# Arshardh/siddhi

Hardware: AMD Instinct MI355X
Metric: events/sec (node) windowed group-by agg at 1/2/4/8 GPUs; % HBM roofline (higher is better)
Workload: dtype f64; 1 GPU; C2 timeBatch(1 sec) count/min/max/avg group by k, per-event sends; key_type=string (dictionary ids = dense slots), keys_per_gpu=100000, keys_total=100000, send_size=1, parallelism=key-sharded x1, flushes=69793, rows=6978983088

## Files before the change

### siddhi_amd/csrc/sh_kernels.hip

```cpp
#include "sh_device.h"

namespace shd {

#ifdef SH_STAMPS
constexpr int kStampKernels = 4, kStampBlocks = 32768, kStampPts = 16;
__device__ unsigned long long g_stamps[kStampKernels * kStampBlocks * kStampPts];
#define SH_STAMP(kern, pt)                                                                                   \
    do {                                                                                                     \
        if (threadIdx.x == 0 && blockIdx.x < kStampBlocks) {                                                 \
            asm volatile("s_waitcnt vmcnt(0) lgkmcnt(0)" ::: "memory");                                      \
            g_stamps[((size_t)(kern) * kStampBlocks + blockIdx.x) * kStampPts + (pt)] = __builtin_amdgcn_s_memtime(); \
        }                                                                                                    \
    } while (0)
#else
#define SH_STAMP(kern, pt) do {} while (0)
#endif

template <int FK>
__global__ __launch_bounds__(kBlock) void k_blockagg(const i64* __restrict__ ts, ColSet cols, FilterProg f,
                                                    WinParams wp, i64* blk_pass, i64* blk_tl, i64* blk_first,
                                                    i64* blk_xm) {
    i64 base = (i64)blockIdx.x * kTile + (i64)threadIdx.x * kItems;
    i64 cnt = 0, tl = INT64_MIN, first = INT64_MAX, xm = INT64_MIN;
    i64 tsv[kItems];
// ... 224 lines not shown
                ms_counts[(i64)(ms_col0 + tile) * P + i] = mhist[i];
        }
    }
    i64 cnt = 0, tl = INT64_MIN;
    SendCursor sc(wp, base);
#pragma unroll
    for (int i = 0; i < kItems; i++) {
        i64 e = base + i;
        bool in = e < wp.N;
        cnt += pass[i];
        if (!SORTED && in && sc.last(wp, e)) tl = max(tl, t[i]);
        sc.next();
    }
    i64 pcb, pm = INT64_MIN;
    if (SORTED) {
        i64 tot_c;
        pcb = block_excl_scan(cnt, SumOp(), 0, &tot_c);
        if (threadIdx.x == 0) blk_pass_pre[tile] = tot_c;
        bool down = false;
#pragma unroll
        for (int i = 0; i + 1 < kItems; i++) down |= base + i + 1 < wp.N && t[i + 1] < t[i];
        if (base + kItems < wp.N) down |= ts[base + kItems] < t[kItems - 1];
        if (down) atomicOr(&info->unsorted, 1);
    } else {
        pcb = block_excl_scan(cnt, SumOp(), 0, nullptr) + blk_pass_pre[tile];
        pm = max(block_excl_scan(tl, MaxOp(), INT64_MIN, nullptr), blk_tl_pre[tile]);
    }
    constexpr bool ext = EXT;
    i64 av[kItems];
    i64 M = INT64_MIN;
    if (ext) {
        load_items_raw(cols, wp.ts_col, base, wp.N, av);
        i64 xm = INT64_MIN;
// ... 86 lines not shown
    int* nb = &info->n_bounds;
#define SH_BOUNDS(EXT, FK, S)                                                                                     \
    hipLaunchKernelGGL((k_boundaries<EXT, FK, S>), dim3(nblk), dim3(kBlock), lds, s, ts, cols, f, wp, blk_pass_pre, \
                       blk_tl_pre, info, bounds, max_bounds, nb, kp, kt, new_pos, blk_xm_pre, ms_counts, P, ms_nblk,   \
                       ms_col0)
    const int fk = filter_kind(f);
    if (wp.kind == SH_WIN_EXT_TIME_BATCH) SH_BOUNDS(true, 2, false);
    else if (sorted) {
        if (fk == 0) SH_BOUNDS(false, 0, true);
        else if (fk == 1) SH_BOUNDS(false, 1, true);
        else SH_BOUNDS(false, 2, true);
    } else if (fk == 0) SH_BOUNDS(false, 0, false);
    else if (fk == 1) SH_BOUNDS(false, 1, false);
    else SH_BOUNDS(false, 2, false);
#undef SH_BOUNDS
    if (sorted) {
        launch_scan_sum_large(s, blk_pass_pre, nblk + 1, scan_tmp);
        hipLaunchKernelGGL(k_fix_bounds, dim3(1), dim3(kBlock), 0, s, bounds, max_bounds, blk_pass_pre, nblk, ts, wp,
                           info);
    }
}

struct AggLds {
    u64* fields;
    u32* cnt;
    u32* first;
    u32* last;
    u32* owner;
};


// ... 1748 lines not shown
```

### siddhi_amd/csrc/sh_runtime.cpp

```cpp
#include <hip/hip_runtime.h>

#include <algorithm>
#include <cstdio>
#include <cstdlib>
#include <cstring>
#include <string>
#include <vector>

#include "sh_agg.h"
#include "sh_internal.h"
#include "sh_runtime.h"

#include <chrono>

using namespace shd;

thread_local std::string g_last_error;

int sh_fail(int code, const std::string& msg) {
    g_last_error = msg;
    SH_TRACE("error %d: %s", code, msg.c_str());
    return code;
}

// ... 128 lines not shown
    HIPCHK(hipSetDevice(device));
    hipDeviceProp_t prop;
    HIPCHK(hipGetDeviceProperties(&prop, device));
    if (std::string(prop.gcnArchName).find("gfx950") == std::string::npos)
        return sh_fail(SH_ERR_DEVICE, std::string("built for gfx950, found ") + prop.gcnArchName);
    hipMemPool_t pool = nullptr;
    if (hipDeviceGetDefaultMemPool(&pool, device) == hipSuccess && pool) {
        uint64_t keep = UINT64_MAX;
        (void)hipMemPoolSetAttribute(pool, hipMemPoolAttrReleaseThreshold, &keep);
    }
    sh_ctx* c = new sh_ctx();
    c->device = device;
    c->num_cus = prop.multiProcessorCount;
    c->max_lds = (int)prop.sharedMemPerBlock;
    if (hipStreamCreateWithFlags(&c->stream, hipStreamNonBlocking) != hipSuccess ||
        hipStreamCreateWithFlags(&c->copy_stream, hipStreamNonBlocking) != hipSuccess) {
        if (c->stream) (void)hipStreamDestroy(c->stream);
        delete c;
        return sh_fail(SH_ERR_DEVICE, "hipStreamCreate failed");
    }
    *out = c;
    return SH_OK;
}

extern "C" int sh_ctx_destroy(sh_ctx* c) {
    if (!c) return SH_OK;
    (void)hipStreamSynchronize(c->stream);
    (void)hipStreamSynchronize(c->copy_stream);
    (void)hipStreamDestroy(c->stream);
    (void)hipStreamDestroy(c->copy_stream);
    delete c;
    return SH_OK;
}

extern "C" int sh_alloc_pinned(int64_t bytes, void** out) {
    if (!out || bytes < 0) return sh_fail(SH_ERR_INVALID, "sh_alloc_pinned: bad arguments");
    HIPCHK(hipHostMalloc(out, (size_t)std::max<int64_t>(bytes, 1), hipHostMallocDefault));
    return SH_OK;
}

extern "C" int sh_free_pinned(void* p) {
    if (p) HIPCHK(hipHostFree(p));
    return SH_OK;
}

extern "C" const char* sh_last_error(void) { return g_last_error.c_str(); }
extern "C" int32_t sh_abi_version(void) { return SH_ABI_VERSION; }

Tuning Tuning::from_env() {
    Tuning t;
    auto on = [](const char* n) { const char* v = getenv(n); return v && *v && strcmp(v, "0") != 0; };
    t.direct_pos = on("SH_DIRECT_POS");
    t.part_keys_1024 = getenv("SH_PART_KEYS") && atoi(getenv("SH_PART_KEYS")) == 1024;
    t.no_async_small = on("SH_NO_ASYNC_SMALL");
    t.sl_records_seq = !getenv("SH_SL_RECORDS_SEQ") || on("SH_SL_RECORDS_SEQ");
    t.pl_sort = !getenv("SH_PL_SORT") || on("SH_PL_SORT");
    if (getenv("SH_AGG_BAND_ROWS")) t.agg_band_rows = atoi(getenv("SH_AGG_BAND_ROWS"));
    t.slx_wave = !getenv("SH_SLX_WAVE") || on("SH_SLX_WAVE");
    return t;
}

extern "C" int sh_query_set_strings(sh_query* q, int32_t col, int64_t first_id, int64_t n, const uint16_t* units,
                                    const int64_t* offsets) {
    if (!q) return sh_fail(SH_ERR_INVALID, "sh_query_set_strings: NULL query");
    if (col < 0 || col >= q->d.n_cols || q->d.col_types[col] != SH_T_STRID)
        return sh_fail(SH_ERR_INVALID, "sh_query_set_strings: not a string column");
    if (first_id < 0 || n < 0 || first_id + n > ((int64_t)1 << 31) || (n > 0 && (!units || !offsets)))
        return sh_fail(SH_ERR_INVALID, "sh_query_set_strings: bad id range");
    for (int64_t i = 0; i < n; i++)
        if (offsets[i + 1] < offsets[i] || offsets[i] < 0)
            return sh_fail(SH_ERR_INVALID, "sh_query_set_strings: offsets must be non-decreasing");
    auto& v = q->strings[col];
    auto& set = q->strings_set[col];
// ... 212 lines not shown
```

### siddhi_amd/csrc/sh_runtime.h

```cpp
#pragma once

#include <hip/hip_runtime.h>
#include <rocprofiler-sdk-roctx/roctx.h>

#include <algorithm>
#include <cstdio>
#include <new>
#include <utility>
#include <string>
#include <unordered_map>
#include <vector>

#include "sh_internal.h"
#include "sh_having.h"

struct sh_ctx {
    int device = 0;
    int num_cus = 0;
    int max_lds = 0;
    hipStream_t stream = nullptr;
    hipStream_t copy_stream = nullptr;
};

int sh_fail(int code, const std::string& msg);

bool sh_trace_on();
#define SH_TRACE(...)                                    \
    do {                                                 \
        if (sh_trace_on()) {                             \
            fprintf(stderr, "[sh] " __VA_ARGS__);        \
            fputc('\n', stderr);                         \
            fflush(stderr);                              \
        }                                                \
    } while (0)

bool sh_timing_on();
// ... 150 lines not shown
    DevBuf blk;
    int stage(hipStream_t s, const sh_batch* b, int n_cols, const int32_t* types, sh_batch* dev);
};

size_t type_size(int t);

using shd::AggPlan;
using shd::FilterProg;
using shd::KeyPlan;
using shd::PushInfo;
using shd::TileMap;

struct SlidingImpl;

struct Tuning {
    bool direct_pos = false, part_keys_1024 = false, no_async_small = false, sl_records_seq = false;
    bool pl_sort = true;
    bool slx_wave = true;
    int agg_band_rows = 8;
    static Tuning from_env();
};

struct WideKeys;
struct sh_query {
    int kind = 0;
    Tuning tune = Tuning::from_env();
    SlidingImpl* sl = nullptr;
    std::unordered_map<int, std::vector<std::u16string>> strings;
    std::unordered_map<int, std::vector<char>> strings_set;
    bool partitioned = false, p0_known = false;
// ... 37 lines not shown
    DevBuf fl_dev;
    HavingState hv;
    std::vector<std::pair<int64_t, int64_t>> xr_starts;
    std::vector<int64_t> xr_rep, xr_vals;
    bool xt_Lvalid = false;
    int64_t xt_L = 0;
    int64_t xt_nnew = 0;
    DevBuf sc_slp, sc_fflag, sc_fo, sc_fc, sc_bclk;
    DevBuf xt_dev;
    PinnedBuf xt_host;
    int64_t n_pend = 0, pend_cap = 0;
    int64_t last_nb = 0;
    int64_t seq = 0;
    DevBuf pend_pos, pend_ts, pend_vals;
    DevBuf pend_tmp;
    DevBuf blk_pass, blk_tl, blk_first, blk_xm, info, bounds, segs, seg_rows, rows, counters, out_ts, out_keys, out_vals,
        out_nulls, out_expired, out_rep, blk_cnt;
    DevBuf first_bits, word_pre;
    DevBuf emit_stage;
    const void* zeroed_nulls = nullptr;
    const void* zeroed_expired = nullptr;
    DevBuf ms_counts, ms_tmp, rec_pos, rec_idx, rec_vals, part_off;
    DevBuf new_pos, seg_off;
    PushInfo* h_info = nullptr;
    PinnedBuf h_up;
    PinnedBuf h_tail;
    PinnedBuf h_bounds;
    bool ms_ready = false;
    bool rec_packed = false;
    bool direct_pos = false;
// ... 18 lines not shown
    int64_t rec_cap = 0;
    struct ClosedTail {
        bool active = false, host_done = false;
        int nseg = 0, units_per_seg = 1;
        int64_t closed_hi = 0;
        std::vector<int64_t> clocks, windows;
    } tail;
    StagedBatch staged;
    OutHost out;
    sh_out dev_out{};
    PinnedVec<int64_t> dev_flush_offsets{0}, dev_flush_clock;
    hipEvent_t ev_push0 = nullptr, ev_push1 = nullptr, ev_agg0 = nullptr, ev_agg1 = nullptr;
    hipEvent_t ev_srt0 = nullptr, ev_srt1 = nullptr;
    bool srt_timed = false;
    hipEvent_t ev_mid = nullptr;
    sh_stats stats{};
    int64_t agg_bytes = 0;
    std::vector<int64_t> flush_window;
    bool internal_keys = false;
    size_t kt_min_size = 0;
    int32_t load_type[SH_MAX_COLS]{};
    uint32_t cols_used = 0;
    bool given = false;
    const int* given_wcol = nullptr;
    const shd::u64* given_gidx = nullptr;
    const int64_t* given_clk = nullptr;
    int64_t given_seq0 = 0, given_ss = 1;
    int64_t given_W_base = 0, given_W_end = 0;
    std::vector<sh_bound> gbounds;
    DevBuf pend_gidx, out_order;
// ... 73 lines not shown
struct FlushVecs {
    PinnedVec<int64_t>& offsets;
    PinnedVec<int64_t>& clocks;
};
inline FlushVecs flush_vecs(sh_query* q, bool host_out) {
    if (host_out) return {q->out.flush_offsets, q->out.flush_clock};
    return {q->dev_flush_offsets, q->dev_flush_clock};
}

int sc_rows(sh_query* q, const sh_batch* b, const std::vector<shd::Bound>& bounds, int64_t n_old, int64_t M, bool cv0,
            int64_t clock0, int64_t seq0, bool host_out);
int sc_expire_pending(sh_query* q, int64_t now, bool host_out);
int hv_closed(sh_query* q, const std::vector<shd::Segment>& segs, const std::vector<int64_t>& clocks, const sh_batch* b,
              bool host_out);
int append_pending(sh_query* q, const sh_batch* b, int64_t n_old, int64_t M);
int upload_segments(sh_query* q, const std::vector<shd::Segment>& segs);

int partition_filter(const FilterProg& base, int pcol, int ptype, int64_t key, FilterProg* out);

int64_t given_flush_clock(const sh_query* q, int64_t W);
int query_push_given(sh_query* q, const sh_batch* b, bool host_out, const sh_out** out);
int query_close_given(sh_query* q, bool host_out, const sh_out** out);
int query_advance(sh_query* q, int64_t now, bool host_out, const sh_out** out);

int query_reserve_keys(sh_query* q, int64_t extra);
int query_drain_async(sh_query* q);
int query_swap_keys(sh_query* q, KeyTableHost& nk);

int sh_query_create_internal(sh_ctx* ctx, const sh_query_desc* d, const KeyPlan& kp, sh_query** out);
int sh_advance_time_device(sh_query* q, int64_t now, const sh_out** out);

// ... 20 lines not shown
```

### siddhi_amd/csrc/sh_window.cpp

```cpp
#include <hip/hip_runtime.h>

#include <algorithm>
#include <atomic>
#include <cstdlib>
#include <cstring>
#include <string>
#include <vector>

#include "sh_agg.h"
#include "sh_internal.h"
#include "sh_runtime.h"
#include "sh_wide.h"

using namespace shd;

#define HIPCHK(x)                                                                                          \
    do {                                                                                                   \
        hipError_t _e = (x);                                                                               \
        if (_e != hipSuccess) return sh_fail(SH_ERR_DEVICE, std::string(#x) + ": " + hipGetErrorString(_e)); \
    } while (0)
#define RCHK(x)            \
    do {                   \
        int _r = (x);      \
        if (_r) return _r; \
// ... 61 lines not shown
    RCHK(nv.reserve(std::max(1, q->ap.n_vcols) * ncap * 8, false));
    RCHK(ng.reserve(ncap * 8, false));
    hipStream_t s = q->ctx->stream;
    if (keep > 0) {
        HIPCHK(hipMemcpyAsync(ng.p, q->pend_gidx.p, keep * 8, hipMemcpyDeviceToDevice, s));
        HIPCHK(hipMemcpyAsync(np.p, q->pend_pos.p, keep * 4, hipMemcpyDeviceToDevice, s));
        HIPCHK(hipMemcpyAsync(nt.p, q->pend_ts.p, keep * 8, hipMemcpyDeviceToDevice, s));
        for (int j = 0; j < q->ap.n_vcols; j++)
            HIPCHK(hipMemcpyAsync((char*)nv.p + j * ncap * 8, (char*)q->pend_vals.p + j * q->pend_cap * 8, keep * 8,
                                  hipMemcpyDeviceToDevice, s));
    }
    HIPCHK(hipStreamSynchronize(s));
    q->pend_pos = std::move(np); q->pend_ts = std::move(nt); q->pend_vals = std::move(nv); q->pend_gidx = std::move(ng);
    q->pend_cap = ncap;
    return SH_OK;
}

static int query_create(sh_ctx* ctx, const sh_query_desc* d, const KeyPlan* kp_override, sh_query** out);
int query_set_partition(sh_query* q, int64_t key);

static bool scatter_fits(const sh_query* q, int p) {
    const int nv = q->ap.n_vcols;
    size_t v = nv <= 1 ? 1 : nv <= 2 ? 2 : nv <= 4 ? 4 : 8;
    return v * kTile * 8 + (size_t)kTile * 8 + (size_t)p * 20 + 64 <= 160 * 1024;
}

static size_t max_table_size(const sh_query* q) {
    int P = 1;
    while (P < 16384 && scatter_fits(q, P << 1)) P <<= 1;
    return (size_t)P * 512;
// ... 225 lines not shown
        q->kind = 1;
        if ((rc = sliding_create(q))) { delete q; return rc; }
        *out = q;
        return SH_OK;
    }
    q->kt_min_size = q->kt.size_;
    if ((rc = size_partitions(q))) { delete q; return rc; }
    if (hipHostMalloc((void**)&q->h_info, sizeof(PushInfo), hipHostMallocDefault) != hipSuccess) {
        delete q;
        return sh_fail(SH_ERR_OOM, "pinned alloc failed");
    }
    if ((rc = q->info.reserve(sizeof(PushInfo), false)) || (rc = q->counters.reserve(64, false))) { delete q; return rc; }
    (void)hipEventCreate(&q->ev_push0); (void)hipEventCreate(&q->ev_push1);
    (void)hipEventCreate(&q->ev_agg0); (void)hipEventCreate(&q->ev_agg1);
    (void)hipEventCreateWithFlags(&q->ev_mid, hipEventDisableTiming);
    *out = q;
    return SH_OK;
}

static bool direct_pos_ok(const sh_query* q) {
    const int kc = q->kp.n == 1 ? q->kp.col[0] : -1;
    return q->kt.dense && q->kt.dmul == 1 && q->kt.dadd == 0 && kc >= 0 && q->kp.div[0] == 0 &&
           (q->load_type[kc] == SH_T_STRID || q->load_type[kc] == SH_T_INT) && filter_kind(q->fp) == 0 &&
           !q->xmode && !q->d.stream_current && q->ap.n > 0 && q->P > 1 && !q->partitioned && !q->given;
}

static bool want_direct_pos(const sh_query* q) {
    return q->tune.direct_pos && direct_pos_ok(q);
}

// ... 21 lines not shown
    wp.kind = q->d.window;
    wp.e0_valid = q->e0_valid;
    wp.clock_valid = q->clock_valid;
    wp.L = wp.T = q->d.window_param;
    wp.cal = q->cal;
    wp.cal_tz = q->cal_tz;
    wp.E0 = q->E0;
    wp.clock0 = q->clock;
    wp.W_open = q->W_open;
    wp.n_pend = q->n_pend;
    wp.send_size = send_size;
    wp.N = N;
    return wp;
}

int upload_segments(sh_query* q, const std::vector<Segment>& segs) {
    const size_t bytes = segs.size() * sizeof(Segment);
    RCHK(q->h_up.reserve(bytes));
    RCHK(q->segs.reserve(bytes, false));
    std::memcpy(q->h_up.p, segs.data(), bytes);
    HIPCHK(hipMemcpyAsync(q->segs.p, q->h_up.p, bytes, hipMemcpyHostToDevice, q->ctx->stream));
    return SH_OK;
}

int append_pending(sh_query* q, const sh_batch* b, int64_t n_old, int64_t M) {
    RCHK(grow_pending(q, M, n_old));
    launch_compact_pending(q->ctx->stream, b->ts, col_set(q, b), pos_src(q, b), q->ap, 0, b->n, 0, n_old,
                           q->blk_pass.as<int64_t>(), q->pend_pos.as<u32>(), q->pend_ts.as<int64_t>(),
                           q->pend_vals.as<u64>(), q->pend_cap, q->given ? q->given_gidx : nullptr,
                           q->pend_gidx.as<u64>(), q->seq);
    HIPCHK(hipGetLastError());
    return SH_OK;
}

static int closed_finish(sh_query* q, bool host_out);

// ... 43 lines not shown
        }
        return SH_OK;
    }
    int64_t row_cap = 0;
    for (auto& sg : segs) row_cap += std::min<int64_t>(sg.hi - sg.lo, (int64_t)q->kt.size_ + 1);
    row_cap = std::max<int64_t>(row_cap, 1);
    const int na = q->ap.n, nk = q->kp.n, RW = row_words(na);
    const int64_t n_words = (closed_hi >> 5) + 1;
    const bool own = q->P > 1 || q->partitioned || closed_hi / nseg >= 65536;
    const int64_t n_units = own ? (int64_t)nseg * q->P : nseg;
    const int unit_stride = agg_unit_rows(q->P, q->NL, own);
    RCHK(q->rows.reserve((size_t)n_units * unit_stride * RW * 8, false));
    RCHK(q->first_bits.reserve((size_t)n_words * 4, false));
    RCHK(q->counters.reserve(64 + (size_t)n_units * 4, false));
    uint32_t* unit_rows = (uint32_t*)(q->counters.as<char>() + 64);
    HIPCHK(hipMemsetAsync(q->first_bits.p, 0, (size_t)n_words * 4, s));
    RCHK(upload_segments(q, segs));
    const Segment* dsegs = q->segs.as<Segment>();
    SH_TRACE("run_closed nseg=%d closed_hi=%lld row_cap=%lld own=%d P=%d NL=%d ms_ready=%d", nseg, (long long)closed_hi,
             (long long)row_cap, (int)own, q->P, q->NL, (int)q->ms_ready);
    if (own) {
        bool long_seg = false;
        for (auto& sg : segs) long_seg |= sg.hi - sg.lo > (int64_t)kPackIdxMask + 1;
        if (q->ms_ready && q->rec_packed && long_seg) q->ms_ready = false;
        if (!q->ms_ready) RCHK(run_multisplit(q, closed_hi, b, false, long_seg));
        RCHK(q->seg_off.reserve((size_t)(nseg + 1) * q->P * 8, false));
        launch_seg_offsets(s, dsegs, nseg, q->n_pend, q->pend_pos.as<u32>(), pos_src(q, b), q->P,
                           q->ms_counts.as<u32>(), q->ms_map, q->seg_off.as<int64_t>());
    }
    const u32* rec_pos = q->rec_pos.as<u32>();
    const u32* rec_idx = q->rec_idx.as<u32>();
    const u64* rec_vals = q->rec_vals.as<u64>();
    const bool gather = own;
    HIPCHK(hipEventRecord(q->ev_agg0, s));
    launch_aggregate(s, dsegs, nseg, q->P, q->logP, q->NL, q->n_pend, q->pend_pos.as<u32>(), q->pend_vals.as<u64>(),
                     q->pend_cap, b ? q->new_pos.as<u32>() : nullptr, cs, q->ap, q->rows.as<u64>(), RW,
                     unit_rows, q->first_bits.as<u32>(),
                     rec_pos, own ? rec_idx : nullptr, rec_vals, (int64_t)q->rec_cap, q->seg_off.as<int64_t>(),
                     q->rec_packed,
                     EvSrc{q->n_pend, q->pend_ts.as<int64_t>(), ts, q->pend_gidx.as<u64>(),
                           q->given && b ? q->given_gidx : nullptr, q->seq},
                     gather);
    HIPCHK(hipGetLastError());
// ... 125 lines not shown

static int close_open_window(sh_query* q, int64_t clock, bool host_out) {
    std::vector<Segment> segs{Segment{0, q->n_pend}};
    std::vector<int64_t> clocks{clock}, windows{q->W_open};
    RCHK(run_closed(q, segs, clocks, windows, nullptr, host_out));
    HIPCHK(hipStreamSynchronize(q->ctx->stream));
    return closed_finish(q, host_out);
}

static void reset_call_output(sh_query* q) {
    q->dev_flush_offsets.assign(1, 0);
    q->dev_flush_clock.clear();
    q->flush_window.clear();
    q->dev_out = sh_out{};
    q->ms_ready = false;
    q->tail.active = false;
}

int flush_layout_to_device(sh_query* q, sh_out& o) {
    if (!q->device_flushes || q->rate.kind != SH_RATE_NONE || q->wide || q->hv.on || !o.flush_offsets) return SH_OK;
    const size_t nf = (size_t)o.n_flushes;
    hipStream_t s = q->ctx->stream;
    RCHK(q->fl_dev.reserve((2 * nf + 1) * 8, false));
    HIPCHK(hipMemcpyAsync(q->fl_dev.p, o.flush_offsets, (nf + 1) * 8, hipMemcpyHostToDevice, s));
    if (nf) HIPCHK(hipMemcpyAsync(q->fl_dev.as<int64_t>() + nf + 1, o.flush_clock, nf * 8, hipMemcpyHostToDevice, s));
    HIPCHK(hipStreamSynchronize(s));
    o.flush_offsets = q->fl_dev.as<int64_t>();
    o.flush_clock = q->fl_dev.as<int64_t>() + nf + 1;
    return SH_OK;
}
// ... 424 lines not shown
static int xr_trim(sh_query* q);
static int push_core(sh_query* q, const sh_batch* b, bool host_out_req, const sh_out** out) {
    SH_TMARK(0);
    const bool host_out = host_out_req && !q->xmode;
    q->x_closes.clear();
    q->x_stamps.clear();
    hipStream_t s = q->ctx->stream;
    q->out.reset();
    reset_call_output(q);
    q->stats = sh_stats{};
    q->agg_bytes = 0;
    q->order_host.clear();
    int64_t N = b->n;
    const bool cv0 = q->clock_valid;
    const int64_t clock0 = q->clock, seq0 = q->seq;
    if (N < 0) return sh_fail(SH_ERR_INVALID, "negative batch size");
    if (N > 0 && (!b->ts)) return sh_fail(SH_ERR_INVALID, "batch without timestamps");
    if (q->n_pend + N >= (int64_t)0xFFFFFFF0ll) return sh_fail(SH_ERR_INVALID, "push larger than 4G events");
    RCHK(small_verify(q, false));
    if (N > 0 && !q->internal_keys && q->kt.n_keys + q->async_keys > (int64_t)q->kt.size_ / 2) {
        RCHK(small_verify(q, true));
        if (q->kt.n_keys > (int64_t)q->kt.size_ / 2) RCHK(query_reserve_keys(q, 0));
    }
    {
        bool done = false;
        RCHK(try_small_push(q, b, &done));
        if (done) return finish_out(q, host_out, out);
        RCHK(small_verify(q, true));
    }
    sh_batch zc_dev;
// ... 13 lines not shown
        WinParams wp = base_win_params(q, b->send_size, N);
        wp.has_start = q->d.has_start_time;
        wp.start_time = q->d.start_time;
        wp.ts_col = q->d.ts_col;
        wp.start_col = q->d.start_col;
        wp.xm0 = q->xm;
        const bool ext = q->d.window == SH_WIN_EXT_TIME_BATCH;
        if (ext) RCHK(q->blk_xm.reserve(nblk * 8, false));
        if (q->given) {
            wp.kind = SH_WIN_TIME_BATCH;
            wp.e0_valid = 1;
            wp.wcol = q->given_wcol;
            wp.W_base = q->given_W_base;
        }
        const bool single_pass = !ext && !q->given && wp.pcol1 == 0 && wp.kind == SH_WIN_TIME_BATCH && wp.e0_valid;
        auto prefix_passes = [&] {
            launch_blockagg(s, b->ts, cs, q->fp, N, b->send_size, q->blk_pass.as<int64_t>(), q->blk_tl.as<int64_t>(),
                            q->blk_first.as<int64_t>(), nblk, ext ? q->blk_xm.as<int64_t>() : nullptr,
                            ext ? q->d.ts_col : -1);
            launch_scan_blocks(s, q->blk_pass.as<int64_t>(), q->blk_tl.as<int64_t>(), q->blk_first.as<int64_t>(), nblk,
                               b->ts, wp, q->info.as<PushInfo>(), ext ? q->blk_xm.as<int64_t>() : nullptr, cs);
        };
        if (single_pass) {
            RCHK(q->blk_pass.reserve((size_t)(nblk + 1) * 8, false));
            launch_zero2(s, q->info.p, (int)sizeof(PushInfo), q->blk_pass.as<int64_t>() + nblk, 8);
            HIPCHK(hipGetLastError());
        } else {
            prefix_passes();
        }
        int max_bounds = (int)std::min<int64_t>(N + 1, 1 << 22);
        RCHK(q->bounds.reserve((size_t)max_bounds * sizeof(Bound), false));
        q->direct_pos = want_direct_pos(q);
        if (!q->direct_pos) RCHK(q->new_pos.reserve((size_t)N * 4, false));
        u32* slot_col = q->direct_pos ? nullptr : q->new_pos.as<u32>();
        const bool early_split = (q->P > 1 || q->partitioned) && N >= (1 << 18) && !q->d.stream_current;
        const TileMap ms_map = make_tile_map(q->n_pend, q->n_pend + N);
        if (early_split) RCHK(reserve_ms_counts(q, ms_map));
        launch_boundaries(s, b->ts, cs, q->fp, wp, q->blk_pass.as<int64_t>(), q->blk_tl.as<int64_t>(),
                          q->info.as<PushInfo>(), q->bounds.as<Bound>(), max_bounds, nblk, q->kp, q->kt.dev(),
                          slot_col, ext ? q->blk_xm.as<int64_t>() : nullptr,
                          early_split ? q->ms_counts.as<u32>() : nullptr, q->P, ms_map.nblk, ms_map.np_t,
                          single_pass, q->blk_tl.as<int64_t>());
        HIPCHK(hipGetLastError());
        constexpr int kFirstBounds = 256;
        const int nb0 = (int)std::min<int64_t>(max_bounds, std::max<int64_t>(kFirstBounds, q->last_nb + q->last_nb / 4 + 64));
        RCHK(q->h_bounds.reserve((size_t)nb0 * sizeof(Bound)));
        HIPCHK(hipMemcpyAsync(q->h_info, q->info.p, sizeof(PushInfo), hipMemcpyDeviceToHost, s));
        HIPCHK(hipMemcpyAsync(q->h_bounds.p, q->bounds.p, (size_t)nb0 * sizeof(Bound), hipMemcpyDeviceToHost, s));
        if (q->band_spec) {
            RCHK(q->h_spec.reserve(16));
            RCHK(q->kt.check_async(s, q->h_spec.as<uint32_t>()));
        }
        HIPCHK(hipEventRecord(q->ev_mid, s));
        SH_TMARK(1);
        if (early_split) RCHK(run_multisplit(q, q->n_pend + N, b, true));
        SH_TRACE("push N=%lld n_pend=%lld: boundaries queued", (long long)N, (long long)q->n_pend);
        SH_TMARK(2);
        if (q->mid_hook) {
            RCHK(q->mid_hook(q->mid_arg));
            SH_TMARK(12);
        }
        HIPCHK(sh_wait_event(q->ev_mid));
        SH_TMARK(3);
        PushInfo info = *q->h_info;
        SH_TRACE("push info: pass=%lld bounds=%d", (long long)info.total_pass, info.n_bounds);
        if (q->band_spec && q->h_spec.as<uint32_t>()[2] == 3) {
            SH_TRACE("push: a bucket outside the speculative key band, retried after a probe");
            return kRetryBand;
        }
        if (single_pass && info.unsorted) {
            SH_TRACE("push: unsorted timestamps, window assignment redone with the prefix passes");
            prefix_passes();
            launch_boundaries(s, b->ts, cs, q->fp, wp, q->blk_pass.as<int64_t>(), q->blk_tl.as<int64_t>(),
                              q->info.as<PushInfo>(), q->bounds.as<Bound>(), max_bounds, nblk, q->kp, q->kt.dev(),
                              slot_col, nullptr);
            HIPCHK(hipGetLastError());
            HIPCHK(hipMemcpyAsync(q->h_info, q->info.p, sizeof(PushInfo), hipMemcpyDeviceToHost, s));
            HIPCHK(hipMemcpyAsync(q->h_bounds.p, q->bounds.p, (size_t)nb0 * sizeof(Bound), hipMemcpyDeviceToHost, s));
            HIPCHK(sh_wait_stream(s));
            info = *q->h_info;
        }
        if (info.n_bounds > max_bounds) return sh_fail(SH_ERR_INVALID, "more than 4M windows closed in one push");
        if (ext && info.err)
            return sh_fail(SH_ERR_UNSUPPORTED,
                           "externalTimeBatch: the first event's timestamp is before its start time (not on the GPU)");
        const int64_t xm0 = q->xm;
        if (ext) q->xm = std::max(q->xm, info.max_xm);
        std::vector<Bound> bounds(info.n_bounds);
        q->last_nb = std::min<int64_t>(info.n_bounds, 1 << 16);
        if (info.n_bounds) {
            if (info.n_bounds <= nb0) {
                std::memcpy(bounds.data(), q->h_bounds.p, info.n_bounds * sizeof(Bound));
            } else {
                HIPCHK(hipMemcpyAsync(bounds.data(), q->bounds.p, info.n_bounds * sizeof(Bound), hipMemcpyDeviceToHost, s));
                HIPCHK(hipStreamSynchronize(s));
            }
            std::sort(bounds.begin(), bounds.end(), [](const Bound& a, const Bound& c) { return a.idx < c.idx; });
        }
        if (q->d.stream_current && q->d.expired_on && q->d.window == SH_WIN_LENGTH_BATCH && !q->given)
            while (!bounds.empty() && bounds.back().pcb >= info.total_pass) bounds.pop_back();
        if (q->xt_replace) {
            RCHK(xr_trim(q));
            for (auto& bd : bounds) q->xr_starts.emplace_back(seq0 + std::max<int64_t>(0, bd.idx - q->n_pend), bd.W);
        }
        if (q->xmode) {
            q->x_stamps.clear();
            if (q->given) {
                given_closes(q);
            } else {
// ... 55 lines not shown
                new_pend = info.total_pass - pcb_lo;
                q->W_open = (!q->given && q->d.window == SH_WIN_LENGTH_BATCH) ? 0 : bounds.back().W;
            }
        } else {
            e_lo = 0;
            pcb_lo = 0;
            dst_base = q->n_pend;
            new_pend = q->n_pend + info.total_pass;
        }
        if (q->d.stream_current) {
            const int64_t n_old = q->n_pend, M = n_old + info.total_pass;
            RCHK(append_pending(q, b, n_old, M));
            if (M > n_old || (q->d.expired_on && !bounds.empty() && n_old > 0))
                RCHK(sc_rows(q, b, bounds, n_old, M, cv0, clock0, seq0, host_out));
            RCHK(pending_to_front(q, M - new_pend, new_pend));
        } else {
            RCHK(grow_pending(q, new_pend, dst_base));
            launch_compact_pending(s, b->ts, cs, pos_src(q, b), q->ap, e_lo, N, pcb_lo, dst_base,
                                   q->blk_pass.as<int64_t>(), q->pend_pos.as<u32>(), q->pend_ts.as<int64_t>(),
                                   q->pend_vals.as<u64>(), q->pend_cap, q->given ? q->given_gidx : nullptr,
                                   q->pend_gidx.as<u64>(), q->seq);
            HIPCHK(hipGetLastError());
        }
        q->n_pend = new_pend;
    }
    q->seq += N;
    HIPCHK(hipEventRecord(q->ev_push1, s));
    RCHK(q->h_tail.reserve(16));
    RCHK(q->kt.check_async(s, q->h_tail.as<uint32_t>()));
    SH_TRACE("push final sync");
    SH_TMARK(4);
    HIPCHK(sh_wait_stream(s));
    SH_TMARK(5);
    SH_TRACE("push done");
    RCHK(q->kt.check_result(q->h_tail.as<uint32_t>()));
    RCHK(closed_finish(q, host_out));
    float ms = 0;
    (void)hipEventElapsedTime(&ms, q->ev_push0, q->ev_push1);
    q->stats.push_ms = ms;
    q->stats.events = N;
    q->stats.main_kernel_bytes = q->agg_bytes;
    if (q->xmode) return xout_finish(q, host_out_req, out);
    RCHK(finish_out(q, host_out, out));
    SH_TMARK(6);
    return SH_OK;
}

int check_batch_cols(const sh_query* q, const sh_batch* b) {
    if (b->n <= 0) return SH_OK;
// ... 288 lines not shown
        return rate_apply(q, *out, false, true, out);
    }
    return advance_core(q, now, true, out);
}

int sh_advance_time_device(sh_query* q, int64_t now, const sh_out** out) {
    return advance_core(q, now, false, out);
}

extern "C" int sh_query_destroy(sh_query* q) {
    StreamScope _ss(q && q->ctx ? q->ctx->stream : nullptr);
    if (!q) return SH_OK;
    (void)small_verify(q, true);
    (void)hipStreamSynchronize(q->ctx->stream);
    (void)hipStreamSynchronize(q->ctx->copy_stream);
    {
        StreamScope none(nullptr);
        for (auto& sl : q->ing.slot) {
            sl.ts.release();
            for (auto& c : sl.cols) c.release();
        }
    }
    ingest_destroy(q);
    if (q->kind == 1) sliding_destroy(q);
    q->kt.release();
    q->gkt.release();
    q->pgkt.release();
    delete q->wide;
    if (q->h_info) (void)hipHostFree(q->h_info);
    if (q->small_res) (void)hipHostFree(q->small_res);
    if (q->zc_ring) (void)hipHostFree(q->zc_ring);
    hipEvent_t evs[] = {q->ev_push0, q->ev_push1, q->ev_agg0, q->ev_agg1, q->ev_mid, q->ev_srt0, q->ev_srt1};
    for (auto e : evs) if (e) (void)hipEventDestroy(e);
    delete q;
    return SH_OK;
}

extern "C" int sh_query_stats(sh_query* q, sh_stats* out) {
    if (!q || !out) return sh_fail(SH_ERR_INVALID, "sh_query_stats: NULL argument");
    *out = q->stats;
    return SH_OK;
}

int reserve_ms_counts(sh_query* q, const TileMap& m) {
    const int64_t ncnt = (int64_t)q->P * (m.nblk + 1);
    RCHK(q->ms_counts.reserve((ncnt + 4) * 4, false));
    return q->ms_tmp.reserve(ms_offsets_tmp_bytes(m.nblk, q->P), false);
}

int run_multisplit(sh_query* q, int64_t hi, const sh_batch* b, bool counted, bool wide) {
    hipStream_t s = q->ctx->stream;
    int P = q->P;
    const ColSet cs = col_set(q, b);
    const TileMap m = counted ? make_tile_map(q->n_pend, hi) : make_tile_map(0, hi);
    RCHK(reserve_ms_counts(q, m));
    RCHK(q->part_off.reserve((P + 1) * 8, false));
    int64_t cap = std::max<int64_t>(hi, 1);
    const bool pack = !wide && q->NL <= 1024;
    if (!pack) RCHK(q->rec_pos.reserve(cap * 4, false));
    RCHK(q->rec_idx.reserve(cap * 4, false));
    RCHK(q->rec_vals.reserve(std::max(1, q->ap.n_vcols) * cap * 8, false));
    const PosSrc np = pos_src(q, b);
    launch_ms_count(s, m, counted ? m.np_t : m.nblk, q->n_pend, q->pend_pos.as<u32>(), np, P, q->ms_counts.as<u32>());
    launch_ms_offsets(s, q->ms_counts.as<u32>(), m.nblk, P, q->ms_tmp.as<int64_t>());
    launch_ms_scatter(s, m, q->n_pend, q->pend_pos.as<u32>(), q->pend_vals.as<u64>(), q->pend_cap, np, cs, q->ap, P,
                      q->logP, q->ms_counts.as<u32>(), pack ? nullptr : q->rec_pos.as<u32>(), q->rec_idx.as<u32>(),
                      q->rec_vals.as<u64>(), cap, pack);
    HIPCHK(hipGetLastError());
    q->ms_ready = true;
    q->rec_packed = pack;
    q->ms_map = m;
    q->rec_cap = cap;
    return SH_OK;
}

static void given_closes(sh_query* q) {
    q->x_closes.clear();
    for (const sh_bound& b : q->gbounds) q->x_closes.emplace_back(b.W, b.clock);
}
// ... 57 lines not shown
```

Before: 33.50 billion events/s.

## Overlap multisplit count, segment offsets and pending compaction on a side stream

Adds a side HIP stream and events so that the pending-row multisplit count, the segment-offset and first-bits setup, and the compaction of pending rows into double-buffered spare buffers run in parallel with the main stream's work. For sorted unfiltered input, the boundaries kernel now writes the per-block pass prefix directly, which removes the block scan, the large scan and the fix-bounds kernel. The info block is packed in front of the boundary array so one device-to-host copy replaces two. In exchange it adds extra buffers and cross-stream event dependencies, which raises the risk of ordering bugs.

```diff
diff --git a/siddhi_amd/csrc/sh_kernels.hip b/siddhi_amd/csrc/sh_kernels.hip
--- a/siddhi_amd/csrc/sh_kernels.hip
+++ b/siddhi_amd/csrc/sh_kernels.hip
@@ -262,9 +262,26 @@
     }
     i64 pcb, pm = INT64_MIN;
     if (SORTED) {
-        i64 tot_c;
-        pcb = block_excl_scan(cnt, SumOp(), 0, &tot_c);
-        if (threadIdx.x == 0) blk_pass_pre[tile] = tot_c;
+        if (FK == 0) {
+            pcb = min(base, wp.N);
+            if (threadIdx.x == 0) {
+                blk_pass_pre[tile] = (i64)tile * kTile;
+                if (tile == (int)gridDim.x - 1) {
+                    blk_pass_pre[gridDim.x] = wp.N;
+                    info->total_pass = wp.N;
+                    info->max_tl = ts[wp.N - 1];
+                    info->first_pass = wp.N ? 0 : INT64_MAX;
+                    info->E0 = wp.E0;
+                    info->e0_valid = wp.e0_valid;
+                    info->first_clk = INT64_MIN;
+                    info->max_xm = INT64_MIN;
+                }
+            }
+        } else {
+            i64 tot_c;
+            pcb = block_excl_scan(cnt, SumOp(), 0, &tot_c);
+            if (threadIdx.x == 0) blk_pass_pre[tile] = tot_c;
+        }
         bool down = false;
 #pragma unroll
         for (int i = 0; i + 1 < kItems; i++) down |= base + i + 1 < wp.N && t[i + 1] < t[i];
@@ -381,7 +398,7 @@
     else if (fk == 1) SH_BOUNDS(false, 1, false);
     else SH_BOUNDS(false, 2, false);
 #undef SH_BOUNDS
-    if (sorted) {
+    if (sorted && fk != 0) {
         launch_scan_sum_large(s, blk_pass_pre, nblk + 1, scan_tmp);
         hipLaunchKernelGGL(k_fix_bounds, dim3(1), dim3(kBlock), 0, s, bounds, max_bounds, blk_pass_pre, nblk, ts, wp,
                            info);
diff --git a/siddhi_amd/csrc/sh_runtime.cpp b/siddhi_amd/csrc/sh_runtime.cpp
--- a/siddhi_amd/csrc/sh_runtime.cpp
+++ b/siddhi_amd/csrc/sh_runtime.cpp
@@ -166,8 +166,10 @@
     c->num_cus = prop.multiProcessorCount;
     c->max_lds = (int)prop.sharedMemPerBlock;
     if (hipStreamCreateWithFlags(&c->stream, hipStreamNonBlocking) != hipSuccess ||
-        hipStreamCreateWithFlags(&c->copy_stream, hipStreamNonBlocking) != hipSuccess) {
+        hipStreamCreateWithFlags(&c->copy_stream, hipStreamNonBlocking) != hipSuccess ||
+        hipStreamCreateWithFlags(&c->side_stream, hipStreamNonBlocking) != hipSuccess) {
         if (c->stream) (void)hipStreamDestroy(c->stream);
+        if (c->copy_stream) (void)hipStreamDestroy(c->copy_stream);
         delete c;
         return sh_fail(SH_ERR_DEVICE, "hipStreamCreate failed");
     }
@@ -179,8 +181,10 @@
     if (!c) return SH_OK;
     (void)hipStreamSynchronize(c->stream);
     (void)hipStreamSynchronize(c->copy_stream);
+    (void)hipStreamSynchronize(c->side_stream);
     (void)hipStreamDestroy(c->stream);
     (void)hipStreamDestroy(c->copy_stream);
+    (void)hipStreamDestroy(c->side_stream);
     delete c;
     return SH_OK;
 }
@@ -209,6 +213,7 @@
     t.pl_sort = !getenv("SH_PL_SORT") || on("SH_PL_SORT");
     if (getenv("SH_AGG_BAND_ROWS")) t.agg_band_rows = atoi(getenv("SH_AGG_BAND_ROWS"));
     t.slx_wave = !getenv("SH_SLX_WAVE") || on("SH_SLX_WAVE");
+    t.side_stream = !getenv("SH_SIDE_STREAM") || on("SH_SIDE_STREAM");
     return t;
 }
 
diff --git a/siddhi_amd/csrc/sh_runtime.h b/siddhi_amd/csrc/sh_runtime.h
--- a/siddhi_amd/csrc/sh_runtime.h
+++ b/siddhi_amd/csrc/sh_runtime.h
@@ -20,6 +20,7 @@
     int max_lds = 0;
     hipStream_t stream = nullptr;
     hipStream_t copy_stream = nullptr;
+    hipStream_t side_stream = nullptr;
 };
 
 int sh_fail(int code, const std::string& msg);
@@ -200,6 +201,7 @@
 struct SlidingImpl;
 
 struct Tuning {
+    bool side_stream = true;
     bool direct_pos = false, part_keys_1024 = false, no_async_small = false, sl_records_seq = false;
     bool pl_sort = true;
     bool slx_wave = true;
@@ -267,6 +269,9 @@
     int64_t seq = 0;
     DevBuf pend_pos, pend_ts, pend_vals;
     DevBuf pend_tmp;
+    DevBuf sp_pos, sp_ts, sp_vals, sp_gidx;
+    int64_t sp_cap = 0;
+    bool side_push = false;
     DevBuf blk_pass, blk_tl, blk_first, blk_xm, info, bounds, segs, seg_rows, rows, counters, out_ts, out_keys, out_vals,
         out_nulls, out_expired, out_rep, blk_cnt;
     DevBuf first_bits, word_pre;
@@ -315,6 +320,7 @@
     hipEvent_t ev_srt0 = nullptr, ev_srt1 = nullptr;
     bool srt_timed = false;
     hipEvent_t ev_mid = nullptr;
+    hipEvent_t ev_cnt = nullptr, ev_ms_off = nullptr, ev_seg = nullptr, ev_cmp = nullptr;
     sh_stats stats{};
     int64_t agg_bytes = 0;
     std::vector<int64_t> flush_window;
@@ -418,7 +424,7 @@
 int hv_closed(sh_query* q, const std::vector<shd::Segment>& segs, const std::vector<int64_t>& clocks, const sh_batch* b,
               bool host_out);
 int append_pending(sh_query* q, const sh_batch* b, int64_t n_old, int64_t M);
-int upload_segments(sh_query* q, const std::vector<shd::Segment>& segs);
+int upload_segments(sh_query* q, const std::vector<shd::Segment>& segs, hipStream_t stream = nullptr);
 
 int partition_filter(const FilterProg& base, int pcol, int ptype, int64_t key, FilterProg* out);
 
diff --git a/siddhi_amd/csrc/sh_window.cpp b/siddhi_amd/csrc/sh_window.cpp
--- a/siddhi_amd/csrc/sh_window.cpp
+++ b/siddhi_amd/csrc/sh_window.cpp
@@ -99,6 +99,33 @@
     q->pend_pos = std::move(np); q->pend_ts = std::move(nt); q->pend_vals = std::move(nv); q->pend_gidx = std::move(ng);
     q->pend_cap = ncap;
     return SH_OK;
+}
+
+static int grow_spare(sh_query* q, int64_t need) {
+    if (need <= q->sp_cap) return SH_OK;
+    int64_t ncap = 2 * std::max<int64_t>(need, std::max(q->pend_cap, q->sp_cap));
+    ncap = std::max<int64_t>(ncap, 4096);
+    for (DevBuf* d : {&q->sp_pos, &q->sp_ts, &q->sp_vals, &q->sp_gidx}) {
+        if (d->p) (void)hipFree(d->p);
+        d->p = nullptr;
+        d->cap = d->used = 0;
+    }
+    q->sp_cap = 0;
+    RCHK(q->sp_pos.reserve(ncap * 4, false));
+    RCHK(q->sp_ts.reserve(ncap * 8, false));
+    RCHK(q->sp_vals.reserve(std::max(1, q->ap.n_vcols) * ncap * 8, false));
+    RCHK(q->sp_gidx.reserve(ncap * 8, false));
+    q->sp_cap = ncap;
+    return SH_OK;
+}
+
+static void swap_pending(sh_query* q) {
+    auto sw = [](DevBuf& a, DevBuf& b) { std::swap(a.p, b.p); std::swap(a.cap, b.cap); std::swap(a.used, b.used); };
+    sw(q->pend_pos, q->sp_pos);
+    sw(q->pend_ts, q->sp_ts);
+    sw(q->pend_vals, q->sp_vals);
+    sw(q->pend_gidx, q->sp_gidx);
+    std::swap(q->pend_cap, q->sp_cap);
 }
 
 static int query_create(sh_ctx* ctx, const sh_query_desc* d, const KeyPlan* kp_override, sh_query** out);
@@ -354,6 +381,8 @@
     (void)hipEventCreate(&q->ev_push0); (void)hipEventCreate(&q->ev_push1);
     (void)hipEventCreate(&q->ev_agg0); (void)hipEventCreate(&q->ev_agg1);
     (void)hipEventCreateWithFlags(&q->ev_mid, hipEventDisableTiming);
+    for (hipEvent_t* e : {&q->ev_cnt, &q->ev_ms_off, &q->ev_seg, &q->ev_cmp})
+        (void)hipEventCreateWithFlags(e, hipEventDisableTiming);
     *out = q;
     return SH_OK;
 }
@@ -405,12 +434,12 @@
     return wp;
 }
 
-int upload_segments(sh_query* q, const std::vector<Segment>& segs) {
+int upload_segments(sh_query* q, const std::vector<Segment>& segs, hipStream_t stream) {
     const size_t bytes = segs.size() * sizeof(Segment);
     RCHK(q->h_up.reserve(bytes));
     RCHK(q->segs.reserve(bytes, false));
     std::memcpy(q->h_up.p, segs.data(), bytes);
-    HIPCHK(hipMemcpyAsync(q->segs.p, q->h_up.p, bytes, hipMemcpyHostToDevice, q->ctx->stream));
+    HIPCHK(hipMemcpyAsync(q->segs.p, q->h_up.p, bytes, hipMemcpyHostToDevice, stream ? stream : q->ctx->stream));
     return SH_OK;
 }
 
@@ -484,19 +513,27 @@
     RCHK(q->first_bits.reserve((size_t)n_words * 4, false));
     RCHK(q->counters.reserve(64 + (size_t)n_units * 4, false));
     uint32_t* unit_rows = (uint32_t*)(q->counters.as<char>() + 64);
-    HIPCHK(hipMemsetAsync(q->first_bits.p, 0, (size_t)n_words * 4, s));
-    RCHK(upload_segments(q, segs));
+    bool long_seg = false;
+    for (auto& sg : segs) long_seg |= sg.hi - sg.lo > (int64_t)kPackIdxMask + 1;
+    if (own && q->ms_ready && q->rec_packed && long_seg) q->ms_ready = false;
+    const bool side = q->side_push && own && q->ms_ready;
+    if (!side) q->side_push = false;
+    hipStream_t s2 = side ? q->ctx->side_stream : s;
+    if (side) HIPCHK(hipStreamWaitEvent(s2, q->ev_ms_off, 0));
+    HIPCHK(hipMemsetAsync(q->first_bits.p, 0, (size_t)n_words * 4, s2));
+    RCHK(upload_segments(q, segs, s2));
     const Segment* dsegs = q->segs.as<Segment>();
     SH_TRACE("run_closed nseg=%d closed_hi=%lld row_cap=%lld own=%d P=%d NL=%d ms_ready=%d", nseg, (long long)closed_hi,
              (long long)row_cap, (int)own, q->P, q->NL, (int)q->ms_ready);
     if (own) {
-        bool long_seg = false;
-        for (auto& sg : segs) long_seg |= sg.hi - sg.lo > (int64_t)kPackIdxMask + 1;
-        if (q->ms_ready && q->rec_packed && long_seg) q->ms_ready = false;
         if (!q->ms_ready) RCHK(run_multisplit(q, closed_hi, b, false, long_seg));
         RCHK(q->seg_off.reserve((size_t)(nseg + 1) * q->P * 8, false));
-        launch_seg_offsets(s, dsegs, nseg, q->n_pend, q->pend_pos.as<u32>(), pos_src(q, b), q->P,
+        launch_seg_offsets(s2, dsegs, nseg, q->n_pend, q->pend_pos.as<u32>(), pos_src(q, b), q->P,
                            q->ms_counts.as<u32>(), q->ms_map, q->seg_off.as<int64_t>());
+    }
+    if (side) {
+        HIPCHK(hipEventRecord(q->ev_seg, s2));
+        HIPCHK(hipStreamWaitEvent(s, q->ev_seg, 0));
     }
     const u32* rec_pos = q->rec_pos.as<u32>();
     const u32* rec_idx = q->rec_idx.as<u32>();
@@ -652,6 +689,7 @@
     q->flush_window.clear();
     q->dev_out = sh_out{};
     q->ms_ready = false;
+    q->side_push = false;
     q->tail.active = false;
 }
 
@@ -1106,6 +1144,7 @@
     int64_t N = b->n;
     const bool cv0 = q->clock_valid;
     const int64_t clock0 = q->clock, seq0 = q->seq;
+    bool swap_spare = false;
     if (N < 0) return sh_fail(SH_ERR_INVALID, "negative batch size");
     if (N > 0 && (!b->ts)) return sh_fail(SH_ERR_INVALID, "batch without timestamps");
     if (q->n_pend + N >= (int64_t)0xFFFFFFF0ll) return sh_fail(SH_ERR_INVALID, "push larger than 4G events");
@@ -1149,45 +1188,58 @@
             wp.W_base = q->given_W_base;
         }
         const bool single_pass = !ext && !q->given && wp.pcol1 == 0 && wp.kind == SH_WIN_TIME_BATCH && wp.e0_valid;
+        int max_bounds = (int)std::min<int64_t>(N + 1, 1 << 22);
+        constexpr size_t kInfoPad = 2 * sizeof(Bound);
+        static_assert(sizeof(PushInfo) <= kInfoPad, "the info block must fit in front of the boundaries");
+        RCHK(q->bounds.reserve(kInfoPad + (size_t)max_bounds * sizeof(Bound), false));
+        PushInfo* const d_info = q->bounds.as<PushInfo>();
+        Bound* const d_bounds = (Bound*)(q->bounds.as<char>() + kInfoPad);
         auto prefix_passes = [&] {
             launch_blockagg(s, b->ts, cs, q->fp, N, b->send_size, q->blk_pass.as<int64_t>(), q->blk_tl.as<int64_t>(),
                             q->blk_first.as<int64_t>(), nblk, ext ? q->blk_xm.as<int64_t>() : nullptr,
                             ext ? q->d.ts_col : -1);
             launch_scan_blocks(s, q->blk_pass.as<int64_t>(), q->blk_tl.as<int64_t>(), q->blk_first.as<int64_t>(), nblk,
-                               b->ts, wp, q->info.as<PushInfo>(), ext ? q->blk_xm.as<int64_t>() : nullptr, cs);
+                               b->ts, wp, d_info, ext ? q->blk_xm.as<int64_t>() : nullptr, cs);
         };
         if (single_pass) {
             RCHK(q->blk_pass.reserve((size_t)(nblk + 1) * 8, false));
-            launch_zero2(s, q->info.p, (int)sizeof(PushInfo), q->blk_pass.as<int64_t>() + nblk, 8);
+            launch_zero2(s, d_info, (int)sizeof(PushInfo), q->blk_pass.as<int64_t>() + nblk, 8);
             HIPCHK(hipGetLastError());
         } else {
             prefix_passes();
         }
-        int max_bounds = (int)std::min<int64_t>(N + 1, 1 << 22);
-        RCHK(q->bounds.reserve((size_t)max_bounds * sizeof(Bound), false));
         q->direct_pos = want_direct_pos(q);
         if (!q->direct_pos) RCHK(q->new_pos.reserve((size_t)N * 4, false));
         u32* slot_col = q->direct_pos ? nullptr : q->new_pos.as<u32>();
         const bool early_split = (q->P > 1 || q->partitioned) && N >= (1 << 18) && !q->d.stream_current;
         const TileMap ms_map = make_tile_map(q->n_pend, q->n_pend + N);
         if (early_split) RCHK(reserve_ms_counts(q, ms_map));
+        q->side_push = early_split && q->tune.side_stream && !q->hv.on && q->ap.n != 0 && !q->given && q->xt_timeout == 0;
         launch_boundaries(s, b->ts, cs, q->fp, wp, q->blk_pass.as<int64_t>(), q->blk_tl.as<int64_t>(),
-                          q->info.as<PushInfo>(), q->bounds.as<Bound>(), max_bounds, nblk, q->kp, q->kt.dev(),
+                          d_info, d_bounds, max_bounds, nblk, q->kp, q->kt.dev(),
                           slot_col, ext ? q->blk_xm.as<int64_t>() : nullptr,
                           early_split ? q->ms_counts.as<u32>() : nullptr, q->P, ms_map.nblk, ms_map.np_t,
                           single_pass, q->blk_tl.as<int64_t>());
         HIPCHK(hipGetLastError());
         constexpr int kFirstBounds = 256;
         const int nb0 = (int)std::min<int64_t>(max_bounds, std::max<int64_t>(kFirstBounds, q->last_nb + q->last_nb / 4 + 64));
-        RCHK(q->h_bounds.reserve((size_t)nb0 * sizeof(Bound)));
-        HIPCHK(hipMemcpyAsync(q->h_info, q->info.p, sizeof(PushInfo), hipMemcpyDeviceToHost, s));
-        HIPCHK(hipMemcpyAsync(q->h_bounds.p, q->bounds.p, (size_t)nb0 * sizeof(Bound), hipMemcpyDeviceToHost, s));
+        const size_t first_bytes = kInfoPad + (size_t)nb0 * sizeof(Bound);
+        RCHK(q->h_bounds.reserve(first_bytes));
+        const Bound* const h_bounds = (const Bound*)(q->h_bounds.as<char>() + kInfoPad);
+        HIPCHK(hipMemcpyAsync(q->h_bounds.p, q->bounds.p, first_bytes, hipMemcpyDeviceToHost, s));
         if (q->band_spec) {
             RCHK(q->h_spec.reserve(16));
             RCHK(q->kt.check_async(s, q->h_spec.as<uint32_t>()));
         }
         HIPCHK(hipEventRecord(q->ev_mid, s));
         SH_TMARK(1);
+        if (q->side_push && ms_map.np_t > 0) {
+            hipStream_t ss = q->ctx->side_stream;
+            HIPCHK(hipStreamWaitEvent(ss, q->ev_push0, 0));
+            launch_ms_count(ss, ms_map, ms_map.np_t, q->n_pend, q->pend_pos.as<u32>(), pos_src(q, b), q->P,
+                            q->ms_counts.as<u32>());
+            HIPCHK(hipEventRecord(q->ev_cnt, ss));
+        }
         if (early_split) RCHK(run_multisplit(q, q->n_pend + N, b, true));
         SH_TRACE("push N=%lld n_pend=%lld: boundaries queued", (long long)N, (long long)q->n_pend);
         SH_TMARK(2);
@@ -1197,6 +1249,7 @@
         }
         HIPCHK(sh_wait_event(q->ev_mid));
         SH_TMARK(3);
+        *q->h_info = *q->h_bounds.as<PushInfo>();
         PushInfo info = *q->h_info;
         SH_TRACE("push info: pass=%lld bounds=%d", (long long)info.total_pass, info.n_bounds);
         if (q->band_spec && q->h_spec.as<uint32_t>()[2] == 3) {
@@ -1207,12 +1260,12 @@
             SH_TRACE("push: unsorted timestamps, window assignment redone with the prefix passes");
             prefix_passes();
             launch_boundaries(s, b->ts, cs, q->fp, wp, q->blk_pass.as<int64_t>(), q->blk_tl.as<int64_t>(),
-                              q->info.as<PushInfo>(), q->bounds.as<Bound>(), max_bounds, nblk, q->kp, q->kt.dev(),
+                              d_info, d_bounds, max_bounds, nblk, q->kp, q->kt.dev(),
                               slot_col, nullptr);
             HIPCHK(hipGetLastError());
-            HIPCHK(hipMemcpyAsync(q->h_info, q->info.p, sizeof(PushInfo), hipMemcpyDeviceToHost, s));
-            HIPCHK(hipMemcpyAsync(q->h_bounds.p, q->bounds.p, (size_t)nb0 * sizeof(Bound), hipMemcpyDeviceToHost, s));
+            HIPCHK(hipMemcpyAsync(q->h_bounds.p, q->bounds.p, first_bytes, hipMemcpyDeviceToHost, s));
             HIPCHK(sh_wait_stream(s));
+            *q->h_info = *q->h_bounds.as<PushInfo>();
             info = *q->h_info;
         }
         if (info.n_bounds > max_bounds) return sh_fail(SH_ERR_INVALID, "more than 4M windows closed in one push");
@@ -1225,9 +1278,9 @@
         q->last_nb = std::min<int64_t>(info.n_bounds, 1 << 16);
         if (info.n_bounds) {
             if (info.n_bounds <= nb0) {
-                std::memcpy(bounds.data(), q->h_bounds.p, info.n_bounds * sizeof(Bound));
+                std::memcpy(bounds.data(), h_bounds, info.n_bounds * sizeof(Bound));
             } else {
-                HIPCHK(hipMemcpyAsync(bounds.data(), q->bounds.p, info.n_bounds * sizeof(Bound), hipMemcpyDeviceToHost, s));
+                HIPCHK(hipMemcpyAsync(bounds.data(), d_bounds, info.n_bounds * sizeof(Bound), hipMemcpyDeviceToHost, s));
                 HIPCHK(hipStreamSynchronize(s));
             }
             std::sort(bounds.begin(), bounds.end(), [](const Bound& a, const Bound& c) { return a.idx < c.idx; });
@@ -1313,6 +1366,17 @@
             if (M > n_old || (q->d.expired_on && !bounds.empty() && n_old > 0))
                 RCHK(sc_rows(q, b, bounds, n_old, M, cv0, clock0, seq0, host_out));
             RCHK(pending_to_front(q, M - new_pend, new_pend));
+        } else if (q->side_push && dst_base == 0) {
+            RCHK(grow_spare(q, new_pend));
+            hipStream_t ss = q->ctx->side_stream;
+            HIPCHK(hipStreamWaitEvent(ss, q->ev_agg0, 0));
+            launch_compact_pending(ss, b->ts, cs, pos_src(q, b), q->ap, e_lo, N, pcb_lo, 0, q->blk_pass.as<int64_t>(),
+                                   q->sp_pos.as<u32>(), q->sp_ts.as<int64_t>(), q->sp_vals.as<u64>(), q->sp_cap, nullptr,
+                                   q->sp_gidx.as<u64>(), q->seq);
+            HIPCHK(hipGetLastError());
+            HIPCHK(hipEventRecord(q->ev_cmp, ss));
+            HIPCHK(hipStreamWaitEvent(s, q->ev_cmp, 0));
+            swap_spare = true;
         } else {
             RCHK(grow_pending(q, new_pend, dst_base));
             launch_compact_pending(s, b->ts, cs, pos_src(q, b), q->ap, e_lo, N, pcb_lo, dst_base,
@@ -1332,6 +1396,8 @@
     HIPCHK(sh_wait_stream(s));
     SH_TMARK(5);
     SH_TRACE("push done");
+    if (swap_spare) swap_pending(q);
+    q->side_push = false;
     RCHK(q->kt.check_result(q->h_tail.as<uint32_t>()));
     RCHK(closed_finish(q, host_out));
     float ms = 0;
@@ -1650,6 +1716,7 @@
     (void)small_verify(q, true);
     (void)hipStreamSynchronize(q->ctx->stream);
     (void)hipStreamSynchronize(q->ctx->copy_stream);
+    (void)hipStreamSynchronize(q->ctx->side_stream);
     {
         StreamScope none(nullptr);
         for (auto& sl : q->ing.slot) {
@@ -1666,7 +1733,8 @@
     if (q->h_info) (void)hipHostFree(q->h_info);
     if (q->small_res) (void)hipHostFree(q->small_res);
     if (q->zc_ring) (void)hipHostFree(q->zc_ring);
-    hipEvent_t evs[] = {q->ev_push0, q->ev_push1, q->ev_agg0, q->ev_agg1, q->ev_mid, q->ev_srt0, q->ev_srt1};
+    hipEvent_t evs[] = {q->ev_push0, q->ev_push1, q->ev_agg0, q->ev_agg1, q->ev_mid, q->ev_srt0, q->ev_srt1,
+                        q->ev_cnt, q->ev_ms_off, q->ev_seg, q->ev_cmp};
     for (auto e : evs) if (e) (void)hipEventDestroy(e);
     delete q;
     return SH_OK;
@@ -1697,8 +1765,11 @@
     RCHK(q->rec_idx.reserve(cap * 4, false));
     RCHK(q->rec_vals.reserve(std::max(1, q->ap.n_vcols) * cap * 8, false));
     const PosSrc np = pos_src(q, b);
-    launch_ms_count(s, m, counted ? m.np_t : m.nblk, q->n_pend, q->pend_pos.as<u32>(), np, P, q->ms_counts.as<u32>());
+    const bool side = counted && q->side_push;
+    if (!side) launch_ms_count(s, m, counted ? m.np_t : m.nblk, q->n_pend, q->pend_pos.as<u32>(), np, P, q->ms_counts.as<u32>());
+    else if (m.np_t > 0) HIPCHK(hipStreamWaitEvent(s, q->ev_cnt, 0));
     launch_ms_offsets(s, q->ms_counts.as<u32>(), m.nblk, P, q->ms_tmp.as<int64_t>());
+    if (side) HIPCHK(hipEventRecord(q->ev_ms_off, s));
     launch_ms_scatter(s, m, q->n_pend, q->pend_pos.as<u32>(), q->pend_vals.as<u64>(), q->pend_cap, np, cs, q->ap, P,
                       q->logP, q->ms_counts.as<u32>(), pack ? nullptr : q->rec_pos.as<u32>(), q->rec_idx.as<u32>(),
                       q->rec_vals.as<u64>(), cap, pack);
```

Result: faster. 34.87 billion events/s, median of 6 (+4.1%).
